# qic999/PCTrans

Hardware: AMD Instinct MI355X
Metric: MSDeformAttn+decoder fwd samples/sec at 512x512, 100 queries (higher is better)
Workload: dtype bf16 decoder (autocast) / f32 MSDeformAttn pixel decoder

## Files before the change

### pctrans_amd/csrc/ffn_fused_split.hip

```cpp
#include <stdlib.h>
#include <type_traits>
#include "msda_win_common.hpp"
#include "launchers.hpp"
#include "split_bf16.hpp"

namespace pct {

constexpr int FF_BLOCK = 256;
constexpr int FF_BM = 128;
constexpr int FF_D = 128;
constexpr int FF_CH = 32;
constexpr int FF_W1ROW = 272;
constexpr int FF_W1PLANE = FF_CH * FF_W1ROW;
constexpr int FF_W2ROW = 80;
constexpr int FF_W2PLANE = FF_D * FF_W2ROW;
constexpr int FF_W2OFF = 3 * FF_W1PLANE;
constexpr int FF_STAGE = 57344;
constexpr int FF_PIECES = FF_STAGE / (FF_BLOCK * 16);
constexpr int FF_HALF = FF_PIECES / 2;
constexpr int FF_LDS = 2 * FF_STAGE + 3 * FF_D * 4;
constexpr int FF_B1OFF = 56832;

__global__ __launch_bounds__(256) void ffn_split_weights_kernel(const float *__restrict__ w1, const float *__restrict__ w2,
                                                                const float *__restrict__ b1, const int F,
                                                                unsigned short *__restrict__ img)
{
  const long long e = ((long long)blockIdx.x * 256 + threadIdx.x) * 2;
  const long long n1 = (long long)F * FF_D;
  const int nch = F / FF_CH;
  unsigned p1, p2, p3;
  if (e < n1) {
    const int u = (int)(e / FF_D), k = (int)(e - (long long)u * FF_D);
    split_bf16x3(w1[e], w1[e + 1], p1, p2, p3);
    const int c = (u / FF_CH + nch - 1) % nch;
    unsigned short *d = img + (size_t)c * (FF_STAGE / 2) + (size_t)(u % FF_CH) * (FF_W1ROW / 2) + k;
    store_planes(d, FF_W1PLANE / 2, p1, p2, p3);
  } else if (e < 2 * n1) {
    const long long e2 = e - n1;
    const int c = (int)(e2 / F), u = (int)(e2 - (long long)c * F);
    split_bf16x3(w2[e2], w2[e2 + 1], p1, p2, p3);
    const int uu = u % FF_CH;
    const int s = uu >> 4, v = uu & 15;
    const int g = v >> 3, h = (v >> 2) & 1, t = v & 3;
    unsigned short *d = img + (size_t)(u / FF_CH) * (FF_STAGE / 2) + (size_t)(FF_W2OFF / 2) + (size_t)c * (FF_W2ROW / 2) +
                        (2 * s + h) * 8 + 4 * g + t;
    store_planes(d, FF_W2PLANE / 2, p1, p2, p3);
  } else if (e < 2 * n1 + F) {
    const int u = (int)(e - 2 * n1);
    float *d = reinterpret_cast<float *>(reinterpret_cast<unsigned char *>(img) + (size_t)(u / FF_CH) * FF_STAGE + FF_B1OFF) + u % FF_CH;
    d[0] = b1[u];
    d[1] = b1[u + 1];
  }
}

__global__ __launch_bounds__(FF_BLOCK, 1) void ffn_fused_split_kernel(
    const float *__restrict__ X, const long long ldx, const unsigned short *__restrict__ img, const int F,
    const float *__restrict__ b2, const float *__restrict__ gamma, const float *__restrict__ beta,
    const float eps, const long long M, float *__restrict__ Y, const long long ldy)
{
  extern __shared__ __attribute__((aligned(16))) unsigned char ff_smem[];
  const int tid = threadIdx.x, lane = tid & 63;
  const int wave = __builtin_amdgcn_readfirstlane(tid >> 6);
  const int r = lane & 31, h = lane >> 5;
  const long long ntiles = (M + FF_BM - 1) / FF_BM;
  const int nch = F / FF_CH;

  const auto img_rsrc = __builtin_amdgcn_make_buffer_rsrc(const_cast<unsigned short *>(img), 0, (int)((long long)nch * FF_STAGE),
                                                          0x00020000);
  auto t_dma = [&](const int piece, const int image, unsigned char *stage) {
    auto *dst = (__attribute__((address_space(3))) void *)(stage + piece * (FF_BLOCK * 16) + wave * 1024);
    __builtin_amdgcn_raw_ptr_buffer_load_lds(img_rsrc, dst, 16, tid * 16, image * FF_STAGE + piece * (FF_BLOCK * 16), 0, 0);
  };

  const int w1_off = r * FF_W1ROW + 16 * h;
  const int w2_off = FF_W2OFF + r * FF_W2ROW + 16 * h;

  auto wait_barrier = [](auto n_tag) {
    constexpr int n = decltype(n_tag)::value;
    static_assert(n >= 0 && n < 16, "vmcnt field");
    __builtin_amdgcn_s_waitcnt(0x70 | n);
    asm volatile("s_barrier" ::: "memory");
  };

#pragma unroll
  for (int p = 0; p < FF_PIECES; ++p) {
    t_dma(p, nch - 1, ff_smem + FF_STAGE);
    t_dma(p, 0, ff_smem);
  }
  if (tid < FF_D) {
    float *par = reinterpret_cast<float *>(ff_smem + 2 * FF_STAGE);
    par[tid] = b2 ? b2[tid] : 0.f;
    par[FF_D + tid] = gamma[tid];
    par[2 * FF_D + tid] = beta[tid];
  }
  wait_barrier(std::integral_constant<int, 0>{});
  int cur = 0;

  i32x4 xraw[16];
  auto x_request = [&](const long long tile, const int s0, const int s1) {
    const long long row0 = tile * FF_BM + 32 * wave;
    const long long left = M - row0;
    const unsigned xbytes = (unsigned)((left < 32 ? (left < 0 ? 0 : left) : 32) * ldx * 4);
    const auto xq = __builtin_amdgcn_make_buffer_rsrc(const_cast<float *>(X + (left > 0 ? row0 : 0) * ldx), 0, (int)xbytes, 0x00020000);
    const int xoff = (int)((r * ldx + 8 * h) * 4);
#pragma unroll
    for (int s = s0; s < s1; ++s) {
      xraw[2 * s] = __builtin_amdgcn_raw_buffer_load_b128(xq, xoff, s * 64, 0);
      xraw[2 * s + 1] = __builtin_amdgcn_raw_buffer_load_b128(xq, xoff, s * 64 + 16, 0);
    }
  };

  bf16x8 xp[8][3];
  f32x16 h_hi, h_lo;
  bf16x8 wa[2][3];
  auto split_x = [&](const int s) {
    split_bf16x3_8(__builtin_bit_cast(f32x4, xraw[2 * s]), __builtin_bit_cast(f32x4, xraw[2 * s + 1]), xp[s]);
  };
  auto w1_frags = [&](const unsigned char *st, const int s) {
#pragma unroll
    for (int p = 0; p < 3; ++p) wa[s & 1][p] = *reinterpret_cast<const bf16x8 *>(st + w1_off + 32 * s + p * FF_W1PLANE);
  };
  auto gemm1_step = [&](const int s) {
    const bf16x8 a1 = wa[s & 1][0], a2 = wa[s & 1][1], a3 = wa[s & 1][2];
    h_lo = __builtin_amdgcn_mfma_f32_32x32x16_bf16(a1, xp[s][2], h_lo, 0, 0, 0);
    h_hi = __builtin_amdgcn_mfma_f32_32x32x16_bf16(a1, xp[s][0], h_hi, 0, 0, 0);
    h_lo = __builtin_amdgcn_mfma_f32_32x32x16_bf16(a3, xp[s][0], h_lo, 0, 0, 0);
    h_lo = __builtin_amdgcn_mfma_f32_32x32x16_bf16(a2, xp[s][1], h_lo, 0, 0, 0);
    h_lo = __builtin_amdgcn_mfma_f32_32x32x16_bf16(a1, xp[s][1], h_lo, 0, 0, 0);
    h_lo = __builtin_amdgcn_mfma_f32_32x32x16_bf16(a2, xp[s][0], h_lo, 0, 0, 0);
  };
  auto first_gemm1 = [&](auto epi) {
    unsigned char *pst = ff_smem + (cur ^ 1) * FF_STAGE;
#pragma unroll
    for (int j = 0; j < 16; ++j) h_hi[j] = h_lo[j] = 0.f;
    w1_frags(pst, 0);
    split_x(0);
    __builtin_amdgcn_sched_barrier(0);
#pragma unroll
    for (int s = 0; s < 8; ++s) {
      if (s < 7) w1_frags(pst, s + 1);
      gemm1_step(s);
      if (s < 7) split_x(s + 1);
      if (s < 7) t_dma(FF_HALF + s, 1 % nch, pst);
      epi(s);
      __builtin_amdgcn_sched_group_barrier(0x100, 3, 0);
#pragma unroll
      for (int i = 0; i < 6; ++i) {
        __builtin_amdgcn_sched_group_barrier(0x008, 1, 0);
        __builtin_amdgcn_sched_group_barrier(0x002, 10, 0);
        if (i == 1 && s < 7) __builtin_amdgcn_sched_group_barrier(0x020, 1, 0);
        if (s >= 4 && i < 4) __builtin_amdgcn_sched_group_barrier(0x040, 1, 0);
      }
      __builtin_amdgcn_sched_barrier(0);
    }
    asm volatile("s_waitcnt lgkmcnt(0)\n\ts_barrier" ::: "memory");
  };

  x_request(blockIdx.x, 0, 8);
  first_gemm1([](int) {});

  for (long long tile = blockIdx.x; tile < ntiles; tile += gridDim.x) {
    const long long row0 = tile * FF_BM + 32 * wave;
    const long long left = M - row0;
    const unsigned xbytes = (unsigned)((left < 32 ? (left < 0 ? 0 : left) : 32) * ldx * 4);
    const auto xr = __builtin_amdgcn_make_buffer_rsrc(const_cast<float *>(X + row0 * ldx), 0, (int)xbytes, 0x00020000);
    f32x16 y_hi[4], y_lo[4];
#pragma unroll
    for (int cb = 0; cb < 4; ++cb)
#pragma unroll
      for (int j = 0; j < 16; ++j) y_hi[cb][j] = y_lo[cb][j] = 0.f;
    f32x4 res[16];

    f32x4 bq[4];
    auto load_bias = [&](const unsigned char *st) {
#pragma unroll
      for (int q = 0; q < 4; ++q) bq[q] = *reinterpret_cast<const f32x4 *>(st + FF_B1OFF + (8 * q + 4 * h) * 4);
    };
    w1_frags(ff_smem + cur * FF_STAGE, 0);
    load_bias(ff_smem + cur * FF_STAGE);

    auto chunk_body = [&](auto last_tag, const int chunk) {
      constexpr bool LAST = decltype(last_tag)::value;
      const unsigned char *st = ff_smem + cur * FF_STAGE;
      unsigned char *nst = ff_smem + (cur ^ 1) * FF_STAGE;
      const int nxt = LAST ? 0 : chunk + 1, nxt2 = (chunk + 2) % nch;
      const f32x16 c_hi = h_hi, c_lo = h_lo;
      if constexpr (!LAST) {
#pragma unroll
        for (int j = 0; j < 16; ++j) h_hi[j] = h_lo[j] = 0.f;
      }
      __builtin_amdgcn_sched_barrier(0);
      unsigned hpw[2][3][4];
      bf16x8 wb[2][3], wc[3];
      auto valu_slice = [&](const int m) {
        const int sg = m >> 2, w = m & 3, q = 2 * sg + (w >> 1), t0 = 2 * (w & 1), j0 = 4 * q + t0;
        const float v0 = fmaxf((c_hi[j0] + c_lo[j0]) + bq[q][t0], 0.f);
        const float v1 = fmaxf((c_hi[j0 + 1] + c_lo[j0 + 1]) + bq[q][t0 + 1], 0.f);
        split_bf16x3(v0, v1, hpw[sg][0][w], hpw[sg][1][w], hpw[sg][2][w]);
      };
      auto h_frag = [&](const int sg, const int p) {
        return __builtin_bit_cast(bf16x8, i32x4{(int)hpw[sg][p][0], (int)hpw[sg][p][1], (int)hpw[sg][p][2], (int)hpw[sg][p][3]});
      };
#pragma unroll
      for (int s = 0; s < 8; ++s) {
        if constexpr (!LAST) {
          if (s < 7) w1_frags(st, s + 1);
          gemm1_step(s);
        }
        if (s == 7) {
#pragma unroll
          for (int p = 0; p < 3; ++p) wb[0][p] = *reinterpret_cast<const bf16x8 *>(st + w2_off + p * FF_W2PLANE);
        }
        if (s & 1) valu_slice(s >> 1);
        if constexpr (LAST) {
          if (s < 6) {
#pragma unroll
            for (int i = s < 4 ? 3 * s : 2 * s + 4; i < (s < 4 ? 3 * s + 3 : 2 * s + 6); ++i)
              res[i] = __builtin_bit_cast(f32x4, __builtin_amdgcn_raw_buffer_load_b128(xr, (int)((r * ldx + 4 * h) * 4), 32 * i, 0));
          }
        }
        if (s < 3) {
          t_dma(2 * s, nxt, nst);
          t_dma(2 * s + 1, nxt, nst);
        }
        if (s == 3) t_dma(6, nxt, nst);
        if constexpr (!LAST) {
#pragma unroll
          for (int i = 0; i < 6; ++i) {
            __builtin_amdgcn_sched_group_barrier(0x008, 1, 0);
            if (s & 1) __builtin_amdgcn_sched_group_barrier(0x002, 4, 0);
            if (!(i & 1)) __builtin_amdgcn_sched_group_barrier(0x100, 1, 0);
            if ((i == 1 || (i == 3 && s < 3)) && s < 4) __builtin_amdgcn_sched_group_barrier(0x020, 1, 0);
          }
        }
        __builtin_amdgcn_sched_barrier(0);
      }
      __builtin_amdgcn_sched_barrier(0);
      auto w2_frags = [&](bf16x8 (&dst)[3], const int g) {
#pragma unroll
        for (int p = 0; p < 3; ++p)
          dst[p] = *reinterpret_cast<const bf16x8 *>(st + w2_off + (g & 3) * 32 * FF_W2ROW + 32 * (g >> 2) + p * FF_W2PLANE);
      };
#pragma unroll
      for (int g = 0; g < 8; ++g) {
        const int sg = g >> 2, cb = g & 3;
        if (g < 5) w2_frags(wb[(g + 1) & 1], g + 1);
        if (g == 5) {
          w2_frags(wb[0], 6);
          w2_frags(wc, 7);
        }
        if (g < 4) valu_slice(4 + g);
        if constexpr (LAST) x_request(tile + gridDim.x, g, g + 1);
        if constexpr (!LAST) {
          if (g == 6) {
#pragma unroll
            for (int p = FF_HALF; p < FF_HALF + 4; ++p) t_dma(p, nxt2, const_cast<unsigned char *>(st));
            w1_frags(nst, 0);
            load_bias(nst);
          }
          if (g == 7)
#pragma unroll
            for (int p = FF_HALF + 4; p < FF_PIECES; ++p) t_dma(p, nxt2, const_cast<unsigned char *>(st));
        }
        const bf16x8 a1 = g == 7 ? wc[0] : wb[g & 1][0], a2 = g == 7 ? wc[1] : wb[g & 1][1], a3 = g == 7 ? wc[2] : wb[g & 1][2];
        y_lo[cb] = __builtin_amdgcn_mfma_f32_32x32x16_bf16(a1, h_frag(sg, 2), y_lo[cb], 0, 0, 0);
        y_hi[cb] = __builtin_amdgcn_mfma_f32_32x32x16_bf16(a1, h_frag(sg, 0), y_hi[cb], 0, 0, 0);
        y_lo[cb] = __builtin_amdgcn_mfma_f32_32x32x16_bf16(a3, h_frag(sg, 0), y_lo[cb], 0, 0, 0);
        y_lo[cb] = __builtin_amdgcn_mfma_f32_32x32x16_bf16(a2, h_frag(sg, 1), y_lo[cb], 0, 0, 0);
        y_lo[cb] = __builtin_amdgcn_mfma_f32_32x32x16_bf16(a1, h_frag(sg, 1), y_lo[cb], 0, 0, 0);
        y_lo[cb] = __builtin_amdgcn_mfma_f32_32x32x16_bf16(a2, h_frag(sg, 0), y_lo[cb], 0, 0, 0);
#pragma unroll
        for (int i = 0; i < 6; ++i) {
          __builtin_amdgcn_sched_group_barrier(0x008, 1, 0);
          if (g < 4) __builtin_amdgcn_sched_group_barrier(0x002, 4, 0);
          if (g < 5 && !(i & 1)) __builtin_amdgcn_sched_group_barrier(0x100, 1, 0);
          if (g == 5) __builtin_amdgcn_sched_group_barrier(0x100, 1, 0);
          if (g == 6 && !LAST) __builtin_amdgcn_sched_group_barrier(0x100, 1, 0);
          if (g == 6 && !LAST && i == 0) __builtin_amdgcn_sched_group_barrier(0x100, 1, 0);
          if (g == 6 && !LAST && i < 4) __builtin_amdgcn_sched_group_barrier(0x020, 1, 0);
          if (g == 7 && !LAST && i < 3) __builtin_amdgcn_sched_group_barrier(0x020, 1, 0);
        }
        __builtin_amdgcn_sched_barrier(0);
        if (g == 5) {
          if constexpr (LAST) wait_barrier(std::integral_constant<int, 12>{});
          else wait_barrier(std::integral_constant<int, 0>{});
          __builtin_amdgcn_sched_barrier(0);
        }
      }
      cur ^= 1;
    };
    for (int chunk = 0; chunk + 1 < nch; ++chunk) chunk_body(std::false_type{}, chunk);
    chunk_body(std::true_type{}, nch - 1);

    const unsigned ybytes = (unsigned)((left < 32 ? (left < 0 ? 0 : left) : 32) * ldy * 4);
    const auto yr = __builtin_amdgcn_make_buffer_rsrc(Y + row0 * ldy, 0, (int)ybytes, 0x00020000);
    float v[64];
#pragma unroll
    for (int cb = 0; cb < 4; ++cb)
#pragma unroll
      for (int q = 0; q < 4; ++q) {
        const int c0 = 32 * cb + 8 * q + 4 * h;
        const f32x4 bb = *reinterpret_cast<const f32x4 *>(ff_smem + 2 * FF_STAGE + c0 * 4);
#pragma unroll
        for (int t = 0; t < 4; ++t) v[16 * cb + 4 * q + t] = ((y_hi[cb][4 * q + t] + y_lo[cb][4 * q + t]) + bb[t]) + res[4 * cb + q][t];
      }
    __builtin_amdgcn_sched_barrier(0);
    float sm = 0.f, s2 = 0.f, mean, rstd;
    auto epi = [&](const int s) {
      if (s < 2) {
#pragma unroll
        for (int j = 32 * s; j < 32 * s + 32; ++j) sm += v[j];
        if (s == 1) {
          sm += __shfl_xor(sm, 32);
          mean = sm * (1.f / 128.f);
        }
      } else if (s < 4) {
#pragma unroll
        for (int j = 32 * (s - 2); j < 32 * (s - 2) + 32; ++j) {
          v[j] -= mean;
          s2 += v[j] * v[j];
        }
        if (s == 3) {
          s2 += __shfl_xor(s2, 32);
          rstd = rsqrtf(s2 * (1.f / 128.f) + eps);
        }
      } else {
        const int cb = s - 4;
#pragma unroll
        for (int q = 0; q < 4; ++q) {
          const int c0 = 32 * cb + 8 * q + 4 * h;
          const f32x4 gq = *reinterpret_cast<const f32x4 *>(ff_smem + 2 * FF_STAGE + (FF_D + c0) * 4);
          const f32x4 eq = *reinterpret_cast<const f32x4 *>(ff_smem + 2 * FF_STAGE + (2 * FF_D + c0) * 4);
          f32x4 o;
#pragma unroll
          for (int t = 0; t < 4; ++t) o[t] = v[16 * cb + 4 * q + t] * rstd * gq[t] + eq[t];
          __builtin_amdgcn_raw_buffer_store_b128(__builtin_bit_cast(i32x4, o), yr, (int)((r * ldy + 4 * h) * 4), 4 * (c0 - 4 * h), 0);
        }
      }
    };
    first_gemm1(epi);
  }
  __builtin_amdgcn_s_waitcnt(0x70);
}

int prepare_ffn_device() { return func_attr_per_device(reinterpret_cast<const void *>(&ffn_fused_split_kernel), FF_LDS) == hipSuccess ? 0 : PCT_ERR_UNSUPPORTED; }

int launch_ffn_fused_split(const float *x, long long ldx, const float *w1, const float *b1, const float *w2, const float *b2,
                           const float *gamma, const float *beta, float eps, int F, long long rows, void *img_ws, float *out,
                           long long ldo, hipStream_t stream)
{
  if (rows <= 0) return 0;
  if (F <= 0 || F % FF_CH) return PCT_ERR_UNSUPPORTED;
  if ((long long)(F / FF_CH) * FF_STAGE > 0x7fffffffLL) return PCT_ERR_UNSUPPORTED;
  if (32LL * (ldx > ldo ? ldx : ldo) * 4 > 0x7fffffffLL) return PCT_ERR_UNSUPPORTED;
  if (func_attr_per_device(reinterpret_cast<const void *>(&ffn_fused_split_kernel), FF_LDS) != hipSuccess) return PCT_ERR_UNSUPPORTED;
  const long long pairs = (long long)F * FF_D + F / 2;
  hipLaunchKernelGGL(ffn_split_weights_kernel, dim3((unsigned)((pairs + 255) / 256)), dim3(256), 0, stream, w1, w2, b1, F,
                     static_cast<unsigned short *>(img_ws));
  const long long ntiles = (rows + FF_BM - 1) / FF_BM;
  const unsigned gx = (unsigned)(ntiles < 256 ? ntiles : 256);
  hipLaunchKernelGGL(ffn_fused_split_kernel, dim3(gx), dim3(FF_BLOCK), FF_LDS, stream, x, ldx,
                     static_cast<const unsigned short *>(img_ws), F, b2, gamma, beta, eps, rows, out, ldo);
  return (int)hipGetLastError();
}

}
```

Baseline: 1454.

## Pack FFN weight image into contiguous per-lane MFMA fragments and move b1 out of stage

```diff
diff --git a/pctrans_amd/csrc/ffn_fused_split.hip b/pctrans_amd/csrc/ffn_fused_split.hip
--- a/pctrans_amd/csrc/ffn_fused_split.hip
+++ b/pctrans_amd/csrc/ffn_fused_split.hip
@@ -10,20 +10,18 @@
 constexpr int FF_BM = 128;
 constexpr int FF_D = 128;
 constexpr int FF_CH = 32;
-constexpr int FF_W1ROW = 272;
-constexpr int FF_W1PLANE = FF_CH * FF_W1ROW;
-constexpr int FF_W2ROW = 80;
-constexpr int FF_W2PLANE = FF_D * FF_W2ROW;
-constexpr int FF_W2OFF = 3 * FF_W1PLANE;
-constexpr int FF_STAGE = 57344;
+constexpr int FF_FRAG = 1024;
+constexpr int FF_W2OFF = 8 * 3 * FF_FRAG;
+constexpr int FF_STAGE = 2 * FF_W2OFF;
 constexpr int FF_PIECES = FF_STAGE / (FF_BLOCK * 16);
 constexpr int FF_HALF = FF_PIECES / 2;
-constexpr int FF_LDS = 2 * FF_STAGE + 3 * FF_D * 4;
-constexpr int FF_B1OFF = 56832;
+constexpr int FF_PAROFF = 2 * FF_STAGE;
+constexpr int FF_B1OFF = FF_PAROFF + 3 * FF_D * 4;
+constexpr int FF_B1TAB = 4096;
+constexpr int FF_WS_CHUNK = 57344;
 
 __global__ __launch_bounds__(256) void ffn_split_weights_kernel(const float *__restrict__ w1, const float *__restrict__ w2,
-                                                                const float *__restrict__ b1, const int F,
-                                                                unsigned short *__restrict__ img)
+                                                                const int F, unsigned short *__restrict__ img)
 {
   const long long e = ((long long)blockIdx.x * 256 + threadIdx.x) * 2;
   const long long n1 = (long long)F * FF_D;
@@ -33,8 +31,8 @@
     const int u = (int)(e / FF_D), k = (int)(e - (long long)u * FF_D);
     split_bf16x3(w1[e], w1[e + 1], p1, p2, p3);
     const int c = (u / FF_CH + nch - 1) % nch;
-    unsigned short *d = img + (size_t)c * (FF_STAGE / 2) + (size_t)(u % FF_CH) * (FF_W1ROW / 2) + k;
-    store_planes(d, FF_W1PLANE / 2, p1, p2, p3);
+    unsigned short *d = img + (size_t)c * (FF_STAGE / 2) + (k >> 4) * (3 * FF_FRAG / 2) + (u % FF_CH + 32 * ((k >> 3) & 1)) * 8 + (k & 7);
+    store_planes(d, FF_FRAG / 2, p1, p2, p3);
   } else if (e < 2 * n1) {
     const long long e2 = e - n1;
     const int c = (int)(e2 / F), u = (int)(e2 - (long long)c * F);
@@ -42,20 +40,16 @@
     const int uu = u % FF_CH;
     const int s = uu >> 4, v = uu & 15;
     const int g = v >> 3, h = (v >> 2) & 1, t = v & 3;
-    unsigned short *d = img + (size_t)(u / FF_CH) * (FF_STAGE / 2) + (size_t)(FF_W2OFF / 2) + (size_t)c * (FF_W2ROW / 2) +
-                        (2 * s + h) * 8 + 4 * g + t;
-    store_planes(d, FF_W2PLANE / 2, p1, p2, p3);
-  } else if (e < 2 * n1 + F) {
-    const int u = (int)(e - 2 * n1);
-    float *d = reinterpret_cast<float *>(reinterpret_cast<unsigned char *>(img) + (size_t)(u / FF_CH) * FF_STAGE + FF_B1OFF) + u % FF_CH;
-    d[0] = b1[u];
-    d[1] = b1[u + 1];
-  }
-}
-
+    unsigned short *d = img + (size_t)(u / FF_CH) * (FF_STAGE / 2) + (size_t)(FF_W2OFF / 2) + (4 * s + c / 32) * (3 * FF_FRAG / 2) +
+                        (c % 32 + 32 * h) * 8 + 4 * g + t;
+    store_planes(d, FF_FRAG / 2, p1, p2, p3);
+  }
+}
+
+template <bool B1_LDS>
 __global__ __launch_bounds__(FF_BLOCK, 1) void ffn_fused_split_kernel(
     const float *__restrict__ X, const long long ldx, const unsigned short *__restrict__ img, const int F,
-    const float *__restrict__ b2, const float *__restrict__ gamma, const float *__restrict__ beta,
+    const float *__restrict__ b1, const float *__restrict__ b2, const float *__restrict__ gamma, const float *__restrict__ beta,
     const float eps, const long long M, float *__restrict__ Y, const long long ldy)
 {
   extern __shared__ __attribute__((aligned(16))) unsigned char ff_smem[];
@@ -72,8 +66,7 @@
     __builtin_amdgcn_raw_ptr_buffer_load_lds(img_rsrc, dst, 16, tid * 16, image * FF_STAGE + piece * (FF_BLOCK * 16), 0, 0);
   };
 
-  const int w1_off = r * FF_W1ROW + 16 * h;
-  const int w2_off = FF_W2OFF + r * FF_W2ROW + 16 * h;
+  const int frag_off = 16 * lane;
 
   auto wait_barrier = [](auto n_tag) {
     constexpr int n = decltype(n_tag)::value;
@@ -84,15 +77,20 @@
 
 #pragma unroll
   for (int p = 0; p < FF_PIECES; ++p) {
-    t_dma(p, nch - 1, ff_smem + FF_STAGE);
+    if (p < FF_HALF) t_dma(p, nch - 1, ff_smem + FF_STAGE);
     t_dma(p, 0, ff_smem);
   }
   if (tid < FF_D) {
-    float *par = reinterpret_cast<float *>(ff_smem + 2 * FF_STAGE);
+    float *par = reinterpret_cast<float *>(ff_smem + FF_PAROFF);
     par[tid] = b2 ? b2[tid] : 0.f;
     par[FF_D + tid] = gamma[tid];
     par[2 * FF_D + tid] = beta[tid];
   }
+  if constexpr (B1_LDS) {
+    float *tab = reinterpret_cast<float *>(ff_smem + FF_B1OFF);
+    for (int i = tid; i < F; i += FF_BLOCK) tab[i] = b1[i];
+  }
+  const auto b1_rsrc = __builtin_amdgcn_make_buffer_rsrc(const_cast<float *>(b1), 0, F * 4, 0x00020000);
   wait_barrier(std::integral_constant<int, 0>{});
   int cur = 0;
 
@@ -118,7 +116,7 @@
   };
   auto w1_frags = [&](const unsigned char *st, const int s) {
 #pragma unroll
-    for (int p = 0; p < 3; ++p) wa[s & 1][p] = *reinterpret_cast<const bf16x8 *>(st + w1_off + 32 * s + p * FF_W1PLANE);
+    for (int p = 0; p < 3; ++p) wa[s & 1][p] = *reinterpret_cast<const bf16x8 *>(st + frag_off + (3 * s + p) * FF_FRAG);
   };
   auto gemm1_step = [&](const int s) {
     const bf16x8 a1 = wa[s & 1][0], a2 = wa[s & 1][1], a3 = wa[s & 1][2];
@@ -141,14 +139,14 @@
       if (s < 7) w1_frags(pst, s + 1);
       gemm1_step(s);
       if (s < 7) split_x(s + 1);
-      if (s < 7) t_dma(FF_HALF + s, 1 % nch, pst);
+      if (s < FF_HALF) t_dma(FF_HALF + s, 1 % nch, pst);
       epi(s);
       __builtin_amdgcn_sched_group_barrier(0x100, 3, 0);
 #pragma unroll
       for (int i = 0; i < 6; ++i) {
         __builtin_amdgcn_sched_group_barrier(0x008, 1, 0);
         __builtin_amdgcn_sched_group_barrier(0x002, 10, 0);
-        if (i == 1 && s < 7) __builtin_amdgcn_sched_group_barrier(0x020, 1, 0);
+        if (i == 1 && s < FF_HALF) __builtin_amdgcn_sched_group_barrier(0x020, 1, 0);
         if (s >= 4 && i < 4) __builtin_amdgcn_sched_group_barrier(0x040, 1, 0);
       }
       __builtin_amdgcn_sched_barrier(0);
@@ -172,12 +170,15 @@
     f32x4 res[16];
 
     f32x4 bq[4];
-    auto load_bias = [&](const unsigned char *st) {
-#pragma unroll
-      for (int q = 0; q < 4; ++q) bq[q] = *reinterpret_cast<const f32x4 *>(st + FF_B1OFF + (8 * q + 4 * h) * 4);
+    auto load_bias = [&](const int chunk) {
+#pragma unroll
+      for (int q = 0; q < 4; ++q) {
+        if constexpr (B1_LDS) bq[q] = *reinterpret_cast<const f32x4 *>(ff_smem + FF_B1OFF + (chunk * FF_CH + 8 * q + 4 * h) * 4);
+        else bq[q] = __builtin_bit_cast(f32x4, __builtin_amdgcn_raw_buffer_load_b128(b1_rsrc, 16 * h, chunk * (FF_CH * 4) + 32 * q, 0));
+      }
     };
     w1_frags(ff_smem + cur * FF_STAGE, 0);
-    load_bias(ff_smem + cur * FF_STAGE);
+    load_bias(0);
 
     auto chunk_body = [&](auto last_tag, const int chunk) {
       constexpr bool LAST = decltype(last_tag)::value;
@@ -209,7 +210,7 @@
         }
         if (s == 7) {
 #pragma unroll
-          for (int p = 0; p < 3; ++p) wb[0][p] = *reinterpret_cast<const bf16x8 *>(st + w2_off + p * FF_W2PLANE);
+          for (int p = 0; p < 3; ++p) wb[0][p] = *reinterpret_cast<const bf16x8 *>(st + frag_off + FF_W2OFF + p * FF_FRAG);
         }
         if (s & 1) valu_slice(s >> 1);
         if constexpr (LAST) {
@@ -219,18 +220,14 @@
               res[i] = __builtin_bit_cast(f32x4, __builtin_amdgcn_raw_buffer_load_b128(xr, (int)((r * ldx + 4 * h) * 4), 32 * i, 0));
           }
         }
-        if (s < 3) {
-          t_dma(2 * s, nxt, nst);
-          t_dma(2 * s + 1, nxt, nst);
-        }
-        if (s == 3) t_dma(6, nxt, nst);
+        if (s < FF_HALF) t_dma(s, nxt, nst);
         if constexpr (!LAST) {
 #pragma unroll
           for (int i = 0; i < 6; ++i) {
             __builtin_amdgcn_sched_group_barrier(0x008, 1, 0);
             if (s & 1) __builtin_amdgcn_sched_group_barrier(0x002, 4, 0);
             if (!(i & 1)) __builtin_amdgcn_sched_group_barrier(0x100, 1, 0);
-            if ((i == 1 || (i == 3 && s < 3)) && s < 4) __builtin_amdgcn_sched_group_barrier(0x020, 1, 0);
+            if (i == 1 && s < FF_HALF) __builtin_amdgcn_sched_group_barrier(0x020, 1, 0);
           }
         }
         __builtin_amdgcn_sched_barrier(0);
@@ -239,7 +236,7 @@
       auto w2_frags = [&](bf16x8 (&dst)[3], const int g) {
 #pragma unroll
         for (int p = 0; p < 3; ++p)
-          dst[p] = *reinterpret_cast<const bf16x8 *>(st + w2_off + (g & 3) * 32 * FF_W2ROW + 32 * (g >> 2) + p * FF_W2PLANE);
+          dst[p] = *reinterpret_cast<const bf16x8 *>(st + frag_off + FF_W2OFF + (3 * g + p) * FF_FRAG);
       };
 #pragma unroll
       for (int g = 0; g < 8; ++g) {
@@ -254,13 +251,13 @@
         if constexpr (!LAST) {
           if (g == 6) {
 #pragma unroll
-            for (int p = FF_HALF; p < FF_HALF + 4; ++p) t_dma(p, nxt2, const_cast<unsigned char *>(st));
+            for (int p = FF_HALF; p < FF_HALF + 3; ++p) t_dma(p, nxt2, const_cast<unsigned char *>(st));
             w1_frags(nst, 0);
-            load_bias(nst);
+            load_bias(nxt);
           }
           if (g == 7)
 #pragma unroll
-            for (int p = FF_HALF + 4; p < FF_PIECES; ++p) t_dma(p, nxt2, const_cast<unsigned char *>(st));
+            for (int p = FF_HALF + 3; p < FF_PIECES; ++p) t_dma(p, nxt2, const_cast<unsigned char *>(st));
         }
         const bf16x8 a1 = g == 7 ? wc[0] : wb[g & 1][0], a2 = g == 7 ? wc[1] : wb[g & 1][1], a3 = g == 7 ? wc[2] : wb[g & 1][2];
         y_lo[cb] = __builtin_amdgcn_mfma_f32_32x32x16_bf16(a1, h_frag(sg, 2), y_lo[cb], 0, 0, 0);
@@ -277,7 +274,7 @@
           if (g == 5) __builtin_amdgcn_sched_group_barrier(0x100, 1, 0);
           if (g == 6 && !LAST) __builtin_amdgcn_sched_group_barrier(0x100, 1, 0);
           if (g == 6 && !LAST && i == 0) __builtin_amdgcn_sched_group_barrier(0x100, 1, 0);
-          if (g == 6 && !LAST && i < 4) __builtin_amdgcn_sched_group_barrier(0x020, 1, 0);
+          if (g == 6 && !LAST && i < 3) __builtin_amdgcn_sched_group_barrier(0x020, 1, 0);
           if (g == 7 && !LAST && i < 3) __builtin_amdgcn_sched_group_barrier(0x020, 1, 0);
         }
         __builtin_amdgcn_sched_barrier(0);
@@ -300,7 +297,7 @@
 #pragma unroll
       for (int q = 0; q < 4; ++q) {
         const int c0 = 32 * cb + 8 * q + 4 * h;
-        const f32x4 bb = *reinterpret_cast<const f32x4 *>(ff_smem + 2 * FF_STAGE + c0 * 4);
+        const f32x4 bb = *reinterpret_cast<const f32x4 *>(ff_smem + FF_PAROFF + c0 * 4);
 #pragma unroll
         for (int t = 0; t < 4; ++t) v[16 * cb + 4 * q + t] = ((y_hi[cb][4 * q + t] + y_lo[cb][4 * q + t]) + bb[t]) + res[4 * cb + q][t];
       }
@@ -329,8 +326,8 @@
 #pragma unroll
         for (int q = 0; q < 4; ++q) {
           const int c0 = 32 * cb + 8 * q + 4 * h;
-          const f32x4 gq = *reinterpret_cast<const f32x4 *>(ff_smem + 2 * FF_STAGE + (FF_D + c0) * 4);
-          const f32x4 eq = *reinterpret_cast<const f32x4 *>(ff_smem + 2 * FF_STAGE + (2 * FF_D + c0) * 4);
+          const f32x4 gq = *reinterpret_cast<const f32x4 *>(ff_smem + FF_PAROFF + (FF_D + c0) * 4);
+          const f32x4 eq = *reinterpret_cast<const f32x4 *>(ff_smem + FF_PAROFF + (2 * FF_D + c0) * 4);
           f32x4 o;
 #pragma unroll
           for (int t = 0; t < 4; ++t) o[t] = v[16 * cb + 4 * q + t] * rstd * gq[t] + eq[t];
@@ -343,7 +340,13 @@
   __builtin_amdgcn_s_waitcnt(0x70);
 }
 
-int prepare_ffn_device() { return func_attr_per_device(reinterpret_cast<const void *>(&ffn_fused_split_kernel), FF_LDS) == hipSuccess ? 0 : PCT_ERR_UNSUPPORTED; }
+static hipError_t ffn_lds_attr()
+{
+  const hipError_t rc = func_attr_per_device(reinterpret_cast<const void *>(&ffn_fused_split_kernel<true>), FF_B1OFF + FF_B1TAB * 4);
+  return rc != hipSuccess ? rc : func_attr_per_device(reinterpret_cast<const void *>(&ffn_fused_split_kernel<false>), FF_B1OFF);
+}
+
+int prepare_ffn_device() { return ffn_lds_attr() == hipSuccess ? 0 : PCT_ERR_UNSUPPORTED; }
 
 int launch_ffn_fused_split(const float *x, long long ldx, const float *w1, const float *b1, const float *w2, const float *b2,
                            const float *gamma, const float *beta, float eps, int F, long long rows, void *img_ws, float *out,
@@ -351,16 +354,20 @@
 {
   if (rows <= 0) return 0;
   if (F <= 0 || F % FF_CH) return PCT_ERR_UNSUPPORTED;
-  if ((long long)(F / FF_CH) * FF_STAGE > 0x7fffffffLL) return PCT_ERR_UNSUPPORTED;
+  if ((long long)(F / FF_CH) * FF_WS_CHUNK > 0x7fffffffLL) return PCT_ERR_UNSUPPORTED;
   if (32LL * (ldx > ldo ? ldx : ldo) * 4 > 0x7fffffffLL) return PCT_ERR_UNSUPPORTED;
-  if (func_attr_per_device(reinterpret_cast<const void *>(&ffn_fused_split_kernel), FF_LDS) != hipSuccess) return PCT_ERR_UNSUPPORTED;
-  const long long pairs = (long long)F * FF_D + F / 2;
-  hipLaunchKernelGGL(ffn_split_weights_kernel, dim3((unsigned)((pairs + 255) / 256)), dim3(256), 0, stream, w1, w2, b1, F,
+  if (ffn_lds_attr() != hipSuccess) return PCT_ERR_UNSUPPORTED;
+  const long long pairs = (long long)F * FF_D;
+  hipLaunchKernelGGL(ffn_split_weights_kernel, dim3((unsigned)((pairs + 255) / 256)), dim3(256), 0, stream, w1, w2, F,
                      static_cast<unsigned short *>(img_ws));
   const long long ntiles = (rows + FF_BM - 1) / FF_BM;
   const unsigned gx = (unsigned)(ntiles < 256 ? ntiles : 256);
-  hipLaunchKernelGGL(ffn_fused_split_kernel, dim3(gx), dim3(FF_BLOCK), FF_LDS, stream, x, ldx,
-                     static_cast<const unsigned short *>(img_ws), F, b2, gamma, beta, eps, rows, out, ldo);
+  if (F <= FF_B1TAB)
+    hipLaunchKernelGGL(ffn_fused_split_kernel<true>, dim3(gx), dim3(FF_BLOCK), FF_B1OFF + F * 4, stream, x, ldx,
+                       static_cast<const unsigned short *>(img_ws), F, b1, b2, gamma, beta, eps, rows, out, ldo);
+  else
+    hipLaunchKernelGGL(ffn_fused_split_kernel<false>, dim3(gx), dim3(FF_BLOCK), FF_B1OFF, stream, x, ldx,
+                       static_cast<const unsigned short *>(img_ws), F, b1, b2, gamma, beta, eps, rows, out, ldo);
   return (int)hipGetLastError();
 }
 
```

Result: slower. 1251 (-14.0%).
